# dohlee/rosettafold-pytorch

Measured on AMD Instinct MI355X. Metric: residues/sec forward (L=256, N=128), higher is better.
Workload: dtype bf16; 1 GPU; BASELINE.json configs[1]: bsz=4/GPU, n_seq=128, L=256, d_msa=384, d_pair=288, 8+5 blocks, 4 encoder layers, random-init weights; global_batch=4, parallelism=batch-sharded x1 (replicated weights), launch=one hipGraph replay per step (validation + input copy outside the graph)

## Files before the change

### rosettafold-pytorch_amd/csrc/favor.hip

```cpp
#include <type_traits>

#include "common.h"

#define FV_DH 64
#define FV_M 266
#define FV_MT 17
#define FV_MPAD 288
#define FV_CTX_LD 592
#define FV_DT 5
#define FV_DROWS 80

struct FavorAttnP {
  const h16_t* qkv;
  const h16_t* pc;
  h16_t* out;
  int64_t x_b, x_o, x_s;
  int64_t x_h;
  int64_t o_b, o_o, o_s;
  int q_off, k_off, v_off;
  int n_o, n_h, nitems;
  int nchunks;
  int dbg;
  float eps;
  float ctx_scale;
};

#ifdef RF_H16_IS_F16
#define FV_CS(x) ((x) * p.ctx_scale)
#else
#define FV_CS(x) (x)
#endif

typedef __attribute__((ext_vector_type(4))) short s16x4;

__device__ __forceinline__ int swz_off(int row, int chunk) { return row * 128 + ((chunk ^ (row & 7)) << 4); }

__device__ __forceinline__ void fv_load_tile(char* smem, int lds_off, const h16_t* g, int64_t stride, int nrows,
                                             int wave, int lane) {
  const int ninstr = nrows * 8 / 64;
  for (int it = wave; it < ninstr; it += 4) {
    const int slot = it * 64 + lane;
    const int row = slot >> 3;
    const int clog = (slot & 7) ^ (row & 7);
    rf_glds16(g + (int64_t)row * stride + clog * 8, smem + lds_off + it * 1024);
  }
}

__device__ __forceinline__ float rbf(float x) { return h2f(f2h(x)); }

__device__ __forceinline__ float fv_mfma_done(float acc_reg) {
  asm volatile("s_nop 7\n\ts_nop 3" : "+v"(acc_reg));
  return acc_reg;
}

union Frag {
  h16x8 v;
  unsigned u[4];
  uint2 h[2];
};

template <int LS, bool SOFTMAX>
__global__ __launch_bounds__(256, 1) void favor_attention_kernel(const FavorAttnP p) {
  constexpr int ST = LS / 64;
  constexpr int NSB = LS / 32;
  constexpr int PC_OFF = 0;
  constexpr int K_OFF = FV_MPAD * 128;
  constexpr int V_OFF = K_OFF + LS * 128;
  constexpr int CTX_OFF = V_OFF + LS * 128;
  constexpr int DIAG_OFF = CTX_OFF + FV_DROWS * FV_CTX_LD;
  constexpr int RED_OFF = DIAG_OFF + LS * 4;
  extern __shared__ __attribute__((aligned(16))) char smem[];
  const int tid = threadIdx.x, lane = tid & 63;
  const int wave = __builtin_amdgcn_readfirstlane(tid >> 6) & 3;
  const int fr = lane & 15, fq = lane >> 4;
  const int nm = wave == 0 ? 5 : 4;
  const int m0t = wave == 0 ? 0 : 5 + 4 * (wave - 1);
  const f32x4 epsv = {p.eps, p.eps, p.eps, p.eps};
  Frag ones;
#pragma unroll
  for (int k = 0; k < 4; ++k) ones.u[k] = fr == 0 ? RF_H16_ONE2 : 0u;

  fv_load_tile(smem, PC_OFF, p.pc, FV_DH, FV_MPAD, wave, lane);
  for (int i = tid; i < FV_DROWS * FV_CTX_LD / 4; i += 256) ((unsigned*)(smem + CTX_OFF))[i] = 0u;

  auto item_base = [&](int item, int64_t& xb, int64_t& ob) {
    const int h = item % p.n_h;
    const int t = item / p.n_h;
    const int o = t % p.n_o, b = t / p.n_o;
    xb = (int64_t)b * p.x_b + (int64_t)o * p.x_o + (int64_t)h * p.x_h;
    ob = (int64_t)b * p.o_b + (int64_t)o * p.o_o + h * FV_DH;
  };

  const int nch = p.nchunks;
  int item = blockIdx.x;
  if (item < p.nitems) {
    int64_t xb, ob;
    item_base(item, xb, ob);
    fv_load_tile(smem, K_OFF, p.qkv + xb + p.k_off, p.x_s, LS, wave, lane);
    fv_load_tile(smem, V_OFF, p.qkv + xb + p.v_off, p.x_s, LS, wave, lane);
  }
  bool first = true;
  for (; item < p.nitems; item += gridDim.x) {
    int64_t xb, ob;
    item_base(item, xb, ob);
    if (first)
      asm volatile("s_waitcnt vmcnt(0)" ::: "memory");
    else
      asm volatile("s_waitcnt vmcnt(%0)" ::"n"(ST * 4) : "memory");
    first = false;
    __syncthreads();
    h16x8 qf[ST][2];
    auto load_q = [&](int chunk) {
#pragma unroll
      for (int t = 0; t < ST; ++t) {
        const int s = chunk * LS + (wave * ST + t) * 16 + fr;
        const h16_t* qrow = p.qkv + xb + p.q_off + (int64_t)s * p.x_s;
#pragma unroll
        for (int kk = 0; kk < 2; ++kk) qf[t][kk] = *(const h16x8*)(qrow + (kk * 4 + fq) * 8);
      }
    };
    load_q(0);

    float gmax = 0.f;
    if constexpr (SOFTMAX) {
      for (int s = tid; s < LS; s += 256) {
        float a = 0.f;
#pragma unroll
        for (int c = 0; c < 8; ++c) {
          const h16x8 x = *(const h16x8*)(smem + K_OFF + s * 128 + c * 16);
#pragma unroll
          for (int e = 0; e < 8; ++e) {
            const float f = h2f((h16_t)x[e]);
            a = fmaf(f, f, a);
          }
        }
        ((float*)(smem + DIAG_OFF))[s] = a * (0.0625f * 1.4426950408889634f);
      }
    }

    h16x8 pf[5][2];
#pragma unroll
    for (int j = 0; j < 5; ++j)
#pragma unroll
      for (int kk = 0; kk < 2; ++kk)
        if (j < nm) pf[j][kk] = *(const h16x8*)(smem + PC_OFF + swz_off((m0t + j) * 16 + fr, kk * 4 + fq));

    if constexpr (SOFTMAX) {
      float mx = -INFINITY;
      for (int u = 0; u < NSB; ++u) {
        h16x8 kf[2][2];
#pragma unroll
        for (int t = 0; t < 2; ++t)
#pragma unroll
          for (int kk = 0; kk < 2; ++kk)
            kf[t][kk] = *(const h16x8*)(smem + K_OFF + swz_off((2 * u + t) * 16 + fr, kk * 4 + fq));
#pragma unroll
        for (int j = 0; j < 5; ++j) {
          if (j < nm) {
            const bool valid = (m0t + j) * 16 + fr < FV_M;
#pragma unroll
            for (int t = 0; t < 2; ++t) {
              f32x4 a = {0.f, 0.f, 0.f, 0.f};
              a = rf_mfma16(kf[t][0], pf[j][0], a, 0, 0, 0);
              a = rf_mfma16(kf[t][1], pf[j][1], a, 0, 0, 0);
              if (valid) mx = fmaxf(mx, fmaxf(fmaxf(a[0], a[1]), fmaxf(a[2], a[3])));
            }
          }
        }
      }
      mx = wave_max(mx);
      if (lane == 0) ((float*)(smem + RED_OFF))[wave] = mx;
      __syncthreads();
      const float* red = (const float*)(smem + RED_OFF);
      gmax = fmaxf(fmaxf(red[0], red[1]), fmaxf(red[2], red[3]));
    }

    f32x4 ctx[5][FV_DT];
#pragma unroll
    for (int j = 0; j < 5; ++j)
#pragma unroll
      for (int i = 0; i < FV_DT; ++i) ctx[j][i] = (f32x4){0.f, 0.f, 0.f, 0.f};
    for (int ck = 0; ck < nch; ++ck) {
    if (ck > 0) {
      __syncthreads();
      fv_load_tile(smem, K_OFF, p.qkv + xb + p.k_off + (int64_t)ck * LS * p.x_s, p.x_s, LS, wave, lane);
      fv_load_tile(smem, V_OFF, p.qkv + xb + p.v_off + (int64_t)ck * LS * p.x_s, p.x_s, LS, wave, lane);
      asm volatile("s_waitcnt vmcnt(0)" ::: "memory");
      __syncthreads();
    }
    for (int u = 0; u < NSB; ++u) {
      h16x8 kf[2][2];
#pragma unroll
      for (int t = 0; t < 2; ++t)
#pragma unroll
        for (int kk = 0; kk < 2; ++kk)
          kf[t][kk] = *(const h16x8*)(smem + K_OFF + swz_off((2 * u + t) * 16 + fr, kk * 4 + fq));
      Frag vf[4];
      {
        const int p4 = fr & 3;
#pragma unroll
        for (int i = 0; i < 4; ++i) {
#pragma unroll
          for (int half = 0; half < 2; ++half) {
            const int row = u * 32 + half * 16 + 4 * fq + (fr >> 2);
            const int off = V_OFF + swz_off(row, i * 2 + (p4 >> 1)) + (p4 & 1) * 8;
            const s16x4 r = __builtin_amdgcn_ds_read_tr16_b64_v4i16((__attribute__((address_space(3))) s16x4*)(smem + off));
            vf[i].h[half] = __builtin_bit_cast(uint2, r);
          }
        }
      }
      f32x4 init[2] = {epsv, epsv};
      if constexpr (SOFTMAX) {
#pragma unroll
        for (int t = 0; t < 2; ++t) {
          const float4 d4 = *(const float4*)(smem + DIAG_OFF + ((2 * u + t) * 16 + 4 * fq) * 4);
          init[t] = (f32x4){-(d4.x + gmax), -(d4.y + gmax), -(d4.z + gmax), -(d4.w + gmax)};
        }
      }
#pragma unroll
      for (int j = 0; j < 5; ++j) {
        if (j < nm) {
          f32x4 a[2];
#pragma unroll
          for (int t = 0; t < 2; ++t) {
            a[t] = rf_mfma16(kf[t][0], pf[j][0], init[t], 0, 0, 0);
            a[t] = rf_mfma16(kf[t][1], pf[j][1], a[t], 0, 0, 0);
          }
          float f[2][4];
#pragma unroll
          for (int t = 0; t < 2; ++t)
#pragma unroll
            for (int r = 0; r < 4; ++r) {
              if constexpr (SOFTMAX)
                f[t][r] = __builtin_amdgcn_exp2f(a[t][r]) + p.eps;
              else
                f[t][r] = fmaxf(a[t][r], p.eps);
            }
          if ((m0t + j) == FV_MT - 1 && fr >= FV_M - 16 * (FV_MT - 1)) {
#pragma unroll
            for (int t = 0; t < 2; ++t)
#pragma unroll
              for (int r = 0; r < 4; ++r) f[t][r] = 0.f;
          }
          Frag kfr;
          kfr.u[0] = rf_pack2_h16(f[0][0], f[0][1]);
          kfr.u[1] = rf_pack2_h16(f[0][2], f[0][3]);
          kfr.u[2] = rf_pack2_h16(f[1][0], f[1][1]);
          kfr.u[3] = rf_pack2_h16(f[1][2], f[1][3]);
#pragma unroll
          for (int i = 0; i < 4; ++i)
            ctx[j][i] = rf_mfma16(kfr.v, vf[i].v, ctx[j][i], 0, 0, 0);
          ctx[j][4] = rf_mfma16(kfr.v, ones.v, ctx[j][4], 0, 0, 0);
        }
      }
    }
    }
#pragma unroll
    for (int j = 0; j < 5; ++j) {
      if (j < nm) {
#pragma unroll
        for (int i = 0; i < FV_DT; ++i) {
          uint2 w;
          w.x = rf_pack2_h16(FV_CS(ctx[j][i][0]), FV_CS(ctx[j][i][1]));
          w.y = rf_pack2_h16(FV_CS(ctx[j][i][2]), FV_CS(ctx[j][i][3]));
          *(uint2*)(smem + CTX_OFF + (i * 16 + fr) * FV_CTX_LD + ((m0t + j) * 16 + 4 * fq) * 2) = w;
        }
      }
    }
    __syncthreads();

    asm volatile("s_waitcnt vmcnt(0)" ::: "memory");
    {
      const int nxt = item + gridDim.x;
      if (nxt < p.nitems) {
        int64_t xb2, ob2;
        item_base(nxt, xb2, ob2);
        fv_load_tile(smem, K_OFF, p.qkv + xb2 + p.k_off, p.x_s, LS, wave, lane);
        fv_load_tile(smem, V_OFF, p.qkv + xb2 + p.v_off, p.x_s, LS, wave, lane);
      }
    }

    f32x4 qinit[ST];
#pragma unroll
    for (int t = 0; t < ST; ++t) qinit[t] = epsv;
    if constexpr (SOFTMAX) {
      float dq[ST], rmax[ST];
#pragma unroll
      for (int t = 0; t < ST; ++t) {
        float a = 0.f;
#pragma unroll
        for (int kk = 0; kk < 2; ++kk)
#pragma unroll
          for (int e = 0; e < 8; ++e) {
            const float f = h2f((h16_t)qf[t][kk][e]);
            a = fmaf(f, f, a);
          }
        a += __shfl_xor(a, 16, 64);
        a += __shfl_xor(a, 32, 64);
        dq[t] = a * (0.0625f * 1.4426950408889634f);
        rmax[t] = -INFINITY;
      }
      for (int j = 0; j < FV_MT; ++j) {
        h16x8 pfr[2];
#pragma unroll
        for (int kk = 0; kk < 2; ++kk) pfr[kk] = *(const h16x8*)(smem + PC_OFF + swz_off(j * 16 + fr, kk * 4 + fq));
#pragma unroll
        for (int t = 0; t < ST; ++t) {
          f32x4 a = {0.f, 0.f, 0.f, 0.f};
          a = rf_mfma16(pfr[0], qf[t][0], a, 0, 0, 0);
          a = rf_mfma16(pfr[1], qf[t][1], a, 0, 0, 0);
#pragma unroll
          for (int r = 0; r < 4; ++r)
            if (j * 16 + 4 * fq + r < FV_M) rmax[t] = fmaxf(rmax[t], a[r]);
        }
      }
#pragma unroll
      for (int t = 0; t < ST; ++t) {
        rmax[t] = fmaxf(rmax[t], __shfl_xor(rmax[t], 16, 64));
        rmax[t] = fmaxf(rmax[t], __shfl_xor(rmax[t], 32, 64));
        const float off = -(dq[t] + rmax[t]);
        qinit[t] = (f32x4){off, off, off, off};
      }
    }
    for (int qc = 0; qc < nch; ++qc) {
    if (qc > 0) load_q(qc);
    f32x4 num[FV_DT][ST];
#pragma unroll
    for (int t = 0; t < ST; ++t)
#pragma unroll
      for (int i = 0; i < FV_DT; ++i) num[i][t] = (f32x4){0.f, 0.f, 0.f, 0.f};
    auto mblock = [&](int u, auto last_tag) {
      constexpr bool LAST = decltype(last_tag)::value;
      float f[2][ST][4];
#pragma unroll
      for (int jj = 0; jj < 2; ++jj) {
        if (LAST && jj == 1) {
#pragma unroll
          for (int t = 0; t < ST; ++t)
#pragma unroll
            for (int r = 0; r < 4; ++r) f[jj][t][r] = 0.f;
        } else {
          const int j = 2 * u + jj;
          h16x8 pfr[2];
#pragma unroll
          for (int kk = 0; kk < 2; ++kk) pfr[kk] = *(const h16x8*)(smem + PC_OFF + swz_off(j * 16 + fr, kk * 4 + fq));
#pragma unroll
          for (int t = 0; t < ST; ++t) {
            f32x4 a = rf_mfma16(pfr[0], qf[t][0], qinit[t], 0, 0, 0);
            a = rf_mfma16(pfr[1], qf[t][1], a, 0, 0, 0);
#pragma unroll
            for (int r = 0; r < 4; ++r) {
              float x;
              if constexpr (SOFTMAX)
                x = __builtin_amdgcn_exp2f(a[r]) + p.eps;
              else
                x = fmaxf(a[r], p.eps);
              if (LAST && 4 * fq + r >= FV_M - 16 * (FV_MT - 1)) x = 0.f;
              f[jj][t][r] = x;
            }
          }
        }
      }
      Frag cf[FV_DT];
#pragma unroll
      for (int i = 0; i < FV_DT; ++i) {
        const char* base = smem + CTX_OFF + (i * 16 + fr) * FV_CTX_LD + (32 * u + 4 * fq) * 2;
        cf[i].h[0] = *(const uint2*)base;
        cf[i].h[1] = *(const uint2*)(base + 32);
      }
#pragma unroll
      for (int t = 0; t < ST; ++t) {
        Frag qfr;
        qfr.u[0] = rf_pack2_h16(f[0][t][0], f[0][t][1]);
        qfr.u[1] = rf_pack2_h16(f[0][t][2], f[0][t][3]);
        qfr.u[2] = rf_pack2_h16(f[1][t][0], f[1][t][1]);
        qfr.u[3] = rf_pack2_h16(f[1][t][2], f[1][t][3]);
#pragma unroll
        for (int i = 0; i < FV_DT; ++i)
          num[i][t] = rf_mfma16(cf[i].v, qfr.v, num[i][t], 0, 0, 0);
      }
    };
    for (int u = 0; u < (FV_MT - 1) / 2; ++u) mblock(u, std::false_type{});
    mblock((FV_MT - 1) / 2, std::true_type{});
#pragma unroll
    for (int t = 0; t < ST; ++t) {
      const float dn = __shfl(fv_mfma_done(num[4][t][0]), fr, 64);
      const float inv = 1.f / dn;
      const int s = qc * LS + (wave * ST + t) * 16 + fr;
      h16_t* orow = p.out + ob + (int64_t)s * p.o_s;
#pragma unroll
      for (int i = 0; i < 4; ++i) {
        uint2 w;
        w.x = rf_pack2_h16(num[i][t][0] * inv, num[i][t][1] * inv);
        w.y = rf_pack2_h16(num[i][t][2] * inv, num[i][t][3] * inv);
        *(uint2*)(orow + i * 16 + 4 * fq) = w;
      }
    }
    }
  }
}

#pragma clang diagnostic ignored "-Winline-asm"
__device__ __forceinline__ void fv_glds_asm(const void* src, unsigned lds_addr) {
  asm volatile("s_mov_b32 m0, %0\n\ts_nop 0\n\tglobal_load_lds_dwordx4 %1, off" ::"s"(lds_addr), "v"(src) : "memory", "m0");
}

__device__ __forceinline__ void fv_lds_barrier() {
  asm volatile("s_waitcnt lgkmcnt(0)" ::: "memory");
  __builtin_amdgcn_s_barrier();
  asm volatile("" ::: "memory");
}

__device__ unsigned long long g_fv_cycles[8];
#define FV_STAMP(slot)                                                   \
  if (prof) {                                                            \
    const unsigned long long now = __builtin_readcyclecounter();         \
    acc_cyc[slot] += now - t_last;                                       \
    t_last = now;                                                        \
  }

template <int LS, bool SOFTMAX>
__global__ __launch_bounds__(512, 1) void favor_attention_kernel8(const FavorAttnP p) {
  constexpr int NSB = LS / 32;
  constexpr int NJ = 3;
  constexpr int STB = LS >= 128 ? LS / 128 : 1;
  constexpr int NWB = LS / (16 * STB);
  constexpr int PC_OFF = 0;
  constexpr int K_OFF = FV_MPAD * 128;
  constexpr int V_OFF = K_OFF + LS * 128;
  constexpr int CTX_OFF = V_OFF + LS * 128;
  constexpr int DIAG_OFF = CTX_OFF + FV_DROWS * FV_CTX_LD;
  constexpr int RED_OFF = DIAG_OFF + LS * 4;
  extern __shared__ __attribute__((aligned(16))) char smem[];
  const int tid = threadIdx.x, lane = tid & 63;
  const int wave = __builtin_amdgcn_readfirstlane(tid >> 6) & 7;
  const int fr = lane & 15, fq = lane >> 4;
  const int nm = wave == 0 ? 3 : 2;
  const int m0t = wave == 0 ? 0 : 1 + 2 * wave;
  const f32x4 epsv = {p.eps, p.eps, p.eps, p.eps};
  Frag ones;
#pragma unroll
  for (int k = 0; k < 4; ++k) ones.u[k] = fr == 0 ? RF_H16_ONE2 : 0u;

  const unsigned lds_base = (unsigned)(uintptr_t)(__attribute__((address_space(3))) char*)smem;
  auto load_tile8 = [&](int lds_off, const h16_t* gp, int64_t stride, auto nrows_tag) {
    constexpr int NI = decltype(nrows_tag)::value * 8 / 64;
    int ln = lane;
    asm volatile("" : "+v"(ln));
    const int dma_row = ln >> 3;
    const int dma_col = ((ln & 7) ^ dma_row) * 8;
    const h16_t* g0 = gp + (int64_t)dma_row * stride + dma_col;
#pragma unroll
    for (int k = 0; k < (NI + 7) / 8; ++k) {
      const int it = wave + 8 * k;
      if (NI % 8 == 0 || it < NI)
        fv_glds_asm(g0 + (int64_t)(8 * it) * stride, __builtin_amdgcn_readfirstlane(lds_base + lds_off + it * 1024));
    }
  };
  constexpr std::integral_constant<int, LS> LS_TAG{};
  load_tile8(PC_OFF, p.pc, FV_DH, std::integral_constant<int, FV_MPAD>{});
  for (int i = tid; i < FV_DROWS * FV_CTX_LD / 4; i += 512) ((unsigned*)(smem + CTX_OFF))[i] = 0u;

  auto item_base = [&](int item, int64_t& xb, int64_t& ob) {
    const int h = item % p.n_h;
    const int t = item / p.n_h;
    const int o = t % p.n_o, b = t / p.n_o;
    xb = (int64_t)b * p.x_b + (int64_t)o * p.x_o + (int64_t)h * p.x_h;
    ob = (int64_t)b * p.o_b + (int64_t)o * p.o_o + h * FV_DH;
  };
  auto ctx_col = [](int tile, int q4) { return ((tile >> 1) * 32 + 8 * q4 + 4 * (tile & 1)) * 2; };
  const int nch = SOFTMAX ? 1 : p.nchunks;
  int item = blockIdx.x;
  if (item < p.nitems) {
    int64_t xb, ob;
    item_base(item, xb, ob);
    load_tile8(K_OFF, p.qkv + xb + p.k_off, p.x_s, LS_TAG);
    load_tile8(V_OFF, p.qkv + xb + p.v_off, p.x_s, LS_TAG);
  }
  bool first = true;
  const bool prof = (RF_DBG(p.dbg) & 8) && wave == ((RF_DBG(p.dbg) >> 4) & 7);
  unsigned long long acc_cyc[7] = {0, 0, 0, 0, 0, 0, 0};
  unsigned long long t_last = prof ? __builtin_readcyclecounter() : 0;
  for (; item < p.nitems; item += gridDim.x) {
    int64_t xb, ob;
    item_base(item, xb, ob);
    asm volatile("" : "+v"(xb), "+v"(ob));
    if (prof) {
      t_last = __builtin_readcyclecounter();
      acc_cyc[6] += 1;
    }
    if (first || wave >= NWB)
      asm volatile("s_waitcnt vmcnt(0)" ::: "memory");
    else
      asm volatile("s_waitcnt vmcnt(%0)" ::"n"(STB * 4) : "memory");
    first = false;
    fv_lds_barrier();
    FV_STAMP(0)
    h16x8 pf[NJ][2];
    {
      int frP = fr, fqP = fq;
      asm volatile("" : "+v"(frP), "+v"(fqP));
#pragma unroll
      for (int j = 0; j < NJ; ++j)
#pragma unroll
        for (int kk = 0; kk < 2; ++kk)
          pf[j][kk] = *(const h16x8*)(smem + PC_OFF + m0t * 2048 + swz_off(frP, kk * 4 + fqP) + (j < nm ? j : 0) * 2048);
    }
    h16x8 qf[STB][2];
    auto load_q = [&](int chunk) {
      int frq = fr, fqq = fq;
      asm volatile("" : "+v"(frq), "+v"(fqq));
      if (wave < NWB) {
#pragma unroll
        for (int t = 0; t < STB; ++t) {
          const int s = chunk * LS + (wave * STB + t) * 16 + frq;
          const h16_t* qrow = p.qkv + xb + p.q_off + (int64_t)s * p.x_s;
#pragma unroll
          for (int kk = 0; kk < 2; ++kk) qf[t][kk] = *(const h16x8*)(qrow + (kk * 4 + fqq) * 8);
        }
      }
    };
    load_q(0);

    float gmax = 0.f;
    if constexpr (SOFTMAX) {
      int frS = fr, fqS = fq;
      asm volatile("" : "+v"(frS), "+v"(fqS));
      for (int s = tid; s < LS; s += 512) {
        float a = 0.f;
#pragma unroll
        for (int c = 0; c < 8; ++c) {
          const h16x8 x = *(const h16x8*)(smem + K_OFF + s * 128 + c * 16);
#pragma unroll
          for (int e = 0; e < 8; ++e) {
            const float f = h2f((h16_t)x[e]);
            a = fmaf(f, f, a);
          }
        }
        ((float*)(smem + DIAG_OFF))[s] = a * (0.0625f * 1.4426950408889634f);
      }
      float mx = -INFINITY;
      for (int u = 0; u < NSB; ++u) {
        h16x8 kf[2][2];
#pragma unroll
        for (int t = 0; t < 2; ++t)
#pragma unroll
          for (int kk = 0; kk < 2; ++kk)
            kf[t][kk] = *(const h16x8*)(smem + K_OFF + swz_off((2 * u + t) * 16 + frS, kk * 4 + fqS));
#pragma unroll
        for (int j = 0; j < NJ; ++j) {
          if (j < nm) {
            const h16x8* pfj = pf[j];
            const bool valid = (m0t + j) != FV_MT - 1 || frS < FV_M - 16 * (FV_MT - 1);
#pragma unroll
            for (int t = 0; t < 2; ++t) {
              f32x4 a = {0.f, 0.f, 0.f, 0.f};
              a = rf_mfma16(kf[t][0], pfj[0], a, 0, 0, 0);
              a = rf_mfma16(kf[t][1], pfj[1], a, 0, 0, 0);
              if (valid) mx = fmaxf(mx, fmaxf(fmaxf(a[0], a[1]), fmaxf(a[2], a[3])));
            }
          }
        }
      }
      mx = wave_max(mx);
      if (lane == 0) ((float*)(smem + RED_OFF))[wave] = mx;
      fv_lds_barrier();
      const float* red = (const float*)(smem + RED_OFF);
      gmax = fmaxf(fmaxf(fmaxf(red[0], red[1]), fmaxf(red[2], red[3])), fmaxf(fmaxf(red[4], red[5]), fmaxf(red[6], red[7])));
    }

    f32x4 ctx[NJ][FV_DT];
#pragma unroll
    for (int j = 0; j < NJ; ++j)
#pragma unroll
      for (int i = 0; i < FV_DT; ++i) ctx[j][i] = (f32x4){0.f, 0.f, 0.f, 0.f};
    for (int ck = 0; ck < nch; ++ck) {
      if (ck > 0) {
        __syncthreads();
        load_tile8(K_OFF, p.qkv + xb + p.k_off + (int64_t)ck * LS * p.x_s, p.x_s, LS_TAG);
        load_tile8(V_OFF, p.qkv + xb + p.v_off + (int64_t)ck * LS * p.x_s, p.x_s, LS_TAG);
        asm volatile("s_waitcnt vmcnt(0)" ::: "memory");
        __syncthreads();
      }
      h16x8 kf[2][2];
      Frag vf[4];
      auto load_sblock = [&](int u, h16x8 (&kfo)[2][2], Frag (&vfo)[4]) {
#pragma unroll
        for (int t = 0; t < 2; ++t)
#pragma unroll
          for (int kk = 0; kk < 2; ++kk)
            kfo[t][kk] = *(const h16x8*)(smem + K_OFF + swz_off((2 * u + t) * 16 + fr, kk * 4 + fq));
        const int p4 = fr & 3;
#pragma unroll
        for (int i = 0; i < 4; ++i) {
#pragma unroll
          for (int half = 0; half < 2; ++half) {
            const int row = u * 32 + half * 16 + 4 * fq + (fr >> 2);
            const int off = V_OFF + swz_off(row, i * 2 + (p4 >> 1)) + (p4 & 1) * 8;
            const s16x4 r = __builtin_amdgcn_ds_read_tr16_b64_v4i16((__attribute__((address_space(3))) s16x4*)(smem + off));
            vfo[i].h[half] = __builtin_bit_cast(uint2, r);
          }
        }
      };
      load_sblock(0, kf, vf);
      for (int u = 0; u < ((RF_DBG(p.dbg) & 1) ? 0 : NSB); ++u) {
        h16x8 kfn[2][2];
        Frag vfn[4];
        load_sblock(u + 1 < NSB ? u + 1 : u, kfn, vfn);
        f32x4 init[2] = {epsv, epsv};
        if constexpr (SOFTMAX) {
#pragma unroll
          for (int t = 0; t < 2; ++t) {
            const float4 d4 = *(const float4*)(smem + DIAG_OFF + ((2 * u + t) * 16 + 4 * fq) * 4);
            init[t] = (f32x4){-(d4.x + gmax), -(d4.y + gmax), -(d4.z + gmax), -(d4.w + gmax)};
          }
        }
#pragma unroll
        for (int j = 0; j < NJ; ++j) {
          if (j < nm) {
            const h16x8* pfj = pf[j];
            f32x4 a[2];
#pragma unroll
            for (int t = 0; t < 2; ++t) {
              a[t] = rf_mfma16(kf[t][0], pfj[0], init[t], 0, 0, 0);
              a[t] = rf_mfma16(kf[t][1], pfj[1], a[t], 0, 0, 0);
            }
            float f[2][4];
#pragma unroll
            for (int t = 0; t < 2; ++t)
#pragma unroll
              for (int r = 0; r < 4; ++r) {
                if constexpr (SOFTMAX)
                  f[t][r] = __builtin_amdgcn_exp2f(a[t][r]) + p.eps;
                else
                  f[t][r] = fmaxf(a[t][r], p.eps);
              }
            if ((m0t + j) == FV_MT - 1 && fr >= FV_M - 16 * (FV_MT - 1)) {
#pragma unroll
              for (int t = 0; t < 2; ++t)
#pragma unroll
                for (int r = 0; r < 4; ++r) f[t][r] = 0.f;
            }
            Frag kfr;
            kfr.u[0] = rf_pack2_h16(f[0][0], f[0][1]);
            kfr.u[1] = rf_pack2_h16(f[0][2], f[0][3]);
            kfr.u[2] = rf_pack2_h16(f[1][0], f[1][1]);
            kfr.u[3] = rf_pack2_h16(f[1][2], f[1][3]);
#pragma unroll
            for (int i = 0; i < 4; ++i)
              ctx[j][i] = rf_mfma16(kfr.v, vf[i].v, ctx[j][i], 0, 0, 0);
            ctx[j][4] = rf_mfma16(kfr.v, ones.v, ctx[j][4], 0, 0, 0);
          }
        }
#pragma unroll
        for (int t = 0; t < 2; ++t)
#pragma unroll
          for (int kk = 0; kk < 2; ++kk) kf[t][kk] = kfn[t][kk];
#pragma unroll
        for (int i = 0; i < 4; ++i) vf[i] = vfn[i];
      }
    }
    FV_STAMP(1)
#pragma unroll
    for (int j = 0; j < NJ; ++j)
      if (j < nm) {
#pragma unroll
        for (int i = 0; i < FV_DT; ++i) {
          uint2 w;
          w.x = rf_pack2_h16(FV_CS(ctx[j][i][0]), FV_CS(ctx[j][i][1]));
          w.y = rf_pack2_h16(FV_CS(ctx[j][i][2]), FV_CS(ctx[j][i][3]));
          *(uint2*)(smem + CTX_OFF + (i * 16 + fr) * FV_CTX_LD + ctx_col(m0t + j, fq)) = w;
        }
      }
    fv_lds_barrier();
    FV_STAMP(2)
    asm volatile("s_waitcnt vmcnt(0)" ::: "memory");
#pragma unroll
    for (int t = 0; t < STB; ++t) {
      asm volatile("" : "+v"(qf[t][0]), "+v"(qf[t][1]));
    }
    {
      const int nxt = item + gridDim.x;
      if (nxt < p.nitems) {
        int64_t xb2, ob2;
        item_base(nxt, xb2, ob2);
        load_tile8(K_OFF, p.qkv + xb2 + p.k_off, p.x_s, LS_TAG);
        load_tile8(V_OFF, p.qkv + xb2 + p.v_off, p.x_s, LS_TAG);
      }
    }
    FV_STAMP(3)
    for (int qc = 0; qc < nch; ++qc) {
      if (qc > 0) {
        load_q(qc);
        asm volatile("s_waitcnt vmcnt(0)" ::: "memory");
#pragma unroll
        for (int t = 0; t < STB; ++t) {
          asm volatile("" : "+v"(qf[t][0]), "+v"(qf[t][1]));
        }
      }
      if (wave < NWB) {
        f32x4 qinit[STB];
#pragma unroll
        for (int t = 0; t < STB; ++t) qinit[t] = epsv;
        if constexpr (SOFTMAX) {
          float dq[STB], rmax[STB];
#pragma unroll
          for (int t = 0; t < STB; ++t) {
            float a = 0.f;
#pragma unroll
            for (int kk = 0; kk < 2; ++kk)
#pragma unroll
              for (int e = 0; e < 8; ++e) {
                const float f = h2f((h16_t)qf[t][kk][e]);
                a = fmaf(f, f, a);
              }
            a += __shfl_xor(a, 16, 64);
            a += __shfl_xor(a, 32, 64);
            dq[t] = a * (0.0625f * 1.4426950408889634f);
            rmax[t] = -INFINITY;
          }
          for (int j = 0; j < FV_MT; ++j) {
            h16x8 pfr[2];
#pragma unroll
            for (int kk = 0; kk < 2; ++kk) pfr[kk] = *(const h16x8*)(smem + PC_OFF + swz_off(j * 16 + fr, kk * 4 + fq));
#pragma unroll
            for (int t = 0; t < STB; ++t) {
              f32x4 a = {0.f, 0.f, 0.f, 0.f};
              a = rf_mfma16(pfr[0], qf[t][0], a, 0, 0, 0);
              a = rf_mfma16(pfr[1], qf[t][1], a, 0, 0, 0);
#pragma unroll
              for (int r = 0; r < 4; ++r)
                if (j * 16 + 4 * fq + r < FV_M) rmax[t] = fmaxf(rmax[t], a[r]);
            }
          }
#pragma unroll
          for (int t = 0; t < STB; ++t) {
            rmax[t] = fmaxf(rmax[t], __shfl_xor(rmax[t], 16, 64));
            rmax[t] = fmaxf(rmax[t], __shfl_xor(rmax[t], 32, 64));
            const float off = -(dq[t] + rmax[t]);
            qinit[t] = (f32x4){off, off, off, off};
          }
        }
        f32x4 num[FV_DT][STB];
#pragma unroll
        for (int t = 0; t < STB; ++t)
#pragma unroll
          for (int i = 0; i < FV_DT; ++i) num[i][t] = (f32x4){0.f, 0.f, 0.f, 0.f};
        auto mblock = [&](int u, auto last_tag) {
          constexpr bool LAST = decltype(last_tag)::value;
          float f[2][STB][4];
#pragma unroll
          for (int jj = 0; jj < 2; ++jj) {
            if (LAST && jj == 1) {
#pragma unroll
              for (int t = 0; t < STB; ++t)
#pragma unroll
                for (int r = 0; r < 4; ++r) f[jj][t][r] = 0.f;
            } else {
              const int j = 2 * u + jj;
              h16x8 pfr[2];
#pragma unroll
              for (int kk = 0; kk < 2; ++kk) pfr[kk] = *(const h16x8*)(smem + PC_OFF + swz_off(j * 16 + fr, kk * 4 + fq));
#pragma unroll
              for (int t = 0; t < STB; ++t) {
                f32x4 a = rf_mfma16(pfr[0], qf[t][0], qinit[t], 0, 0, 0);
                a = rf_mfma16(pfr[1], qf[t][1], a, 0, 0, 0);
#pragma unroll
                for (int r = 0; r < 4; ++r) {
                  float x;
                  if constexpr (SOFTMAX)
                    x = __builtin_amdgcn_exp2f(a[r]) + p.eps;
                  else
                    x = fmaxf(a[r], p.eps);
                  if (LAST && 4 * fq + r >= FV_M - 16 * (FV_MT - 1)) x = 0.f;
                  f[jj][t][r] = x;
                }
              }
            }
          }
          Frag cf[FV_DT];
#pragma unroll
          for (int i = 0; i < FV_DT; ++i)
            cf[i].v = *(const h16x8*)(smem + CTX_OFF + (i * 16 + fr) * FV_CTX_LD + (32 * u + 8 * fq) * 2);
#pragma unroll
          for (int t = 0; t < STB; ++t) {
            Frag qfr;
            qfr.u[0] = rf_pack2_h16(f[0][t][0], f[0][t][1]);
            qfr.u[1] = rf_pack2_h16(f[0][t][2], f[0][t][3]);
            qfr.u[2] = rf_pack2_h16(f[1][t][0], f[1][t][1]);
            qfr.u[3] = rf_pack2_h16(f[1][t][2], f[1][t][3]);
#pragma unroll
            for (int i = 0; i < FV_DT; ++i)
              num[i][t] = rf_mfma16(cf[i].v, qfr.v, num[i][t], 0, 0, 0);
          }
        };
        for (int u = 0; u < ((RF_DBG(p.dbg) & 2) ? 0 : (FV_MT - 1) / 2); ++u) mblock(u, std::false_type{});
        mblock((FV_MT - 1) / 2, std::true_type{});
        FV_STAMP(4)
#pragma unroll
        for (int t = 0; t < STB; ++t) {
          const float dn = __shfl(fv_mfma_done(num[4][t][0]), fr, 64);
          const float inv = 1.f / dn;
          const int s = qc * LS + (wave * STB + t) * 16 + fr;
          h16_t* orow = p.out + ob + (int64_t)s * p.o_s;
#pragma unroll
          for (int i = 0; i < 4; ++i) {
            uint2 w;
            w.x = rf_pack2_h16(num[i][t][0] * inv, num[i][t][1] * inv);
            w.y = rf_pack2_h16(num[i][t][2] * inv, num[i][t][3] * inv);
            *(uint2*)(orow + i * 16 + 4 * fq) = w;
          }
        }
      }
    }
    FV_STAMP(5)
  }
  if (prof && lane == 0) {
#pragma unroll
    for (int i = 0; i < 7; ++i) atomicAdd(&g_fv_cycles[i], acc_cyc[i]);
  }
}

extern "C" int rf_favor_phase_cycles(unsigned long long* out7, int reset) {
  unsigned long long z[8] = {0, 0, 0, 0, 0, 0, 0, 0};
  if (out7 && hipMemcpyFromSymbol(out7, HIP_SYMBOL(g_fv_cycles), 7 * sizeof(unsigned long long)) != hipSuccess) return 1000 + (int)hipGetLastError();
  if (reset && hipMemcpyToSymbol(HIP_SYMBOL(g_fv_cycles), z, sizeof(z)) != hipSuccess) return 1000 + (int)hipGetLastError();
  return 0;
}

template <int LS, bool SM>
static int launch_favor(const FavorAttnP& p, hipStream_t s) {
  const size_t lds = (size_t)FV_MPAD * 128 + 2 * (size_t)LS * 128 + (size_t)FV_DROWS * FV_CTX_LD + LS * 4 + 64;
  const int ncu = rf_num_cus() > 0 ? rf_num_cus() : 256;
  const int grid = p.nitems < ncu ? p.nitems : ncu;
  static const bool force4 = getenv("RF_FAVOR4") != nullptr;
  constexpr bool only4 = SM && LS > 128;
  if (only4 || force4) {
    auto k = favor_attention_kernel<LS, SM>;
    if (const int e = rf_enable_big_lds<favor_attention_kernel<LS, SM>>()) return e;
    hipLaunchKernelGGL(k, dim3(grid), dim3(256), lds, s, p);
  } else if constexpr (!only4) {
    auto k = favor_attention_kernel8<LS, SM>;
    if (const int e = rf_enable_big_lds<favor_attention_kernel8<LS, SM>>()) return e;
    hipLaunchKernelGGL(k, dim3(grid), dim3(512), lds, s, p);
  }
  return rf_launch_status();
}

extern "C" int rf_favor_attention(const void* qkv, const void* pc, void* out, const int64_t x_strides[4],
                                  const int64_t o_strides[3], int q_off, int k_off, int v_off, int n_b, int n_o,
                                  int n_h, int seq_len, int dim_head, int n_features, int softmax_kernel, float eps,
                                  void* stream) {
  if (dim_head != FV_DH || n_features != FV_M) return RF_EINVAL;
  int nchunks = 1, ls = seq_len;
  if (seq_len > 256) {
    if (softmax_kernel || seq_len % 256) return RF_EINVAL;
    nchunks = seq_len / 256;
    ls = 256;
  }
  if (ls != 64 && ls != 128 && ls != 256) return RF_EINVAL;
  if (((uintptr_t)qkv % 16) || ((uintptr_t)pc % 16) || ((uintptr_t)out % 8)) return RF_EALIGN;
  for (int i = 0; i < 3; ++i)
    if (x_strides[i] % 8 || o_strides[i] % 4) return RF_EALIGN;
  if (x_strides[3] % 8) return RF_EALIGN;
  if (q_off % 8 || k_off % 8 || v_off % 8) return RF_EALIGN;
  FavorAttnP p;
  p.qkv = (const h16_t*)qkv;
  p.pc = (const h16_t*)pc;
  p.out = (h16_t*)out;
  p.x_b = x_strides[0]; p.x_o = x_strides[1]; p.x_s = x_strides[2]; p.x_h = x_strides[3];
  p.o_b = o_strides[0]; p.o_o = o_strides[1]; p.o_s = o_strides[2];
  p.q_off = q_off; p.k_off = k_off; p.v_off = v_off;
  p.n_o = n_o; p.n_h = n_h;
  p.nitems = n_b * n_o * n_h;
  p.eps = eps;
  p.nchunks = nchunks;
  p.ctx_scale = 1.0f;
#ifdef RF_H16_IS_F16
  for (int n = 1; n < seq_len; n <<= 1) p.ctx_scale *= 0.5f;
#endif
  static int dbg = 0;
  static const int dbg_rc = rf_dbg_env("RF_FAVOR_DBG", &dbg);
  if (dbg_rc) return dbg_rc;
  p.dbg = dbg;
  hipStream_t s = (hipStream_t)stream;
  if (ls == 256) return softmax_kernel ? launch_favor<256, true>(p, s) : launch_favor<256, false>(p, s);
  if (ls == 128) return softmax_kernel ? launch_favor<128, true>(p, s) : launch_favor<128, false>(p, s);
  return softmax_kernel ? launch_favor<64, true>(p, s) : launch_favor<64, false>(p, s);
}
```

Before: 3199 residues/s.

## Cache softmax-path random-feature logits in registers instead of recomputing MFMAs

In the softmax (FAVOR+ positive features) path, the key-side logits computed during the max-finding pass are now kept in registers (zk) and reused in the context accumulation, so the second set of key projection MFMAs is dropped. The query side likewise keeps its logits (zq) from the row-max pass and reuses them in the numerator loop, which is fully unrolled with compile-time indices. The key diagonal norm computation is also spread across 8 lanes per row with shuffle reductions. The softmax branch now handles only a single chunk and no longer contains the multi-chunk reload loop. The cost is much higher register pressure from the large cached accumulator arrays, which could cause spills or lower occupancy.

```diff
diff --git a/rosettafold-pytorch_amd/csrc/favor.hip b/rosettafold-pytorch_amd/csrc/favor.hip
--- a/rosettafold-pytorch_amd/csrc/favor.hip
+++ b/rosettafold-pytorch_amd/csrc/favor.hip
@@ -1,4 +1,5 @@
 #include <type_traits>
+#include <utility>
 
 #include "common.h"
 
@@ -51,6 +52,11 @@
 __device__ __forceinline__ float fv_mfma_done(float acc_reg) {
   asm volatile("s_nop 7\n\ts_nop 3" : "+v"(acc_reg));
   return acc_reg;
+}
+
+template <int... I, class F>
+__device__ __forceinline__ void fv_static_for(std::integer_sequence<int, I...>, F&& f) {
+  (f(std::integral_constant<int, I>{}), ...);
 }
 
 union Frag {
@@ -522,142 +528,205 @@
     };
     load_q(0);
 
-    float gmax = 0.f;
+    f32x4 ctx[NJ][FV_DT];
+#pragma unroll
+    for (int j = 0; j < NJ; ++j)
+#pragma unroll
+      for (int i = 0; i < FV_DT; ++i) ctx[j][i] = (f32x4){0.f, 0.f, 0.f, 0.f};
+    auto load_kblock = [&](int u, int frK, int fqK, h16x8 (&kfo)[2][2]) {
+#pragma unroll
+      for (int t = 0; t < 2; ++t)
+#pragma unroll
+        for (int kk = 0; kk < 2; ++kk)
+          kfo[t][kk] = *(const h16x8*)(smem + K_OFF + swz_off((2 * u + t) * 16 + frK, kk * 4 + fqK));
+    };
+    auto load_vblock = [&](int u, Frag (&vfo)[4]) {
+      const int p4 = fr & 3;
+#pragma unroll
+      for (int i = 0; i < 4; ++i) {
+#pragma unroll
+        for (int half = 0; half < 2; ++half) {
+          const int row = u * 32 + half * 16 + 4 * fq + (fr >> 2);
+          const int off = V_OFF + swz_off(row, i * 2 + (p4 >> 1)) + (p4 & 1) * 8;
+          const s16x4 r = __builtin_amdgcn_ds_read_tr16_b64_v4i16((__attribute__((address_space(3))) s16x4*)(smem + off));
+          vfo[i].h[half] = __builtin_bit_cast(uint2, r);
+        }
+      }
+    };
+    auto ctx_step = [&](int j, float (&f)[2][4], const Frag (&vfu)[4]) {
+      if ((m0t + j) == FV_MT - 1 && fr >= FV_M - 16 * (FV_MT - 1)) {
+#pragma unroll
+        for (int t = 0; t < 2; ++t)
+#pragma unroll
+          for (int r = 0; r < 4; ++r) f[t][r] = 0.f;
+      }
+      Frag kfr;
+      kfr.u[0] = rf_pack2_h16(f[0][0], f[0][1]);
+      kfr.u[1] = rf_pack2_h16(f[0][2], f[0][3]);
+      kfr.u[2] = rf_pack2_h16(f[1][0], f[1][1]);
+      kfr.u[3] = rf_pack2_h16(f[1][2], f[1][3]);
+#pragma unroll
+      for (int i = 0; i < 4; ++i)
+        ctx[j][i] = rf_mfma16(kfr.v, vfu[i].v, ctx[j][i], 0, 0, 0);
+      ctx[j][4] = rf_mfma16(kfr.v, ones.v, ctx[j][4], 0, 0, 0);
+    };
     if constexpr (SOFTMAX) {
-      int frS = fr, fqS = fq;
-      asm volatile("" : "+v"(frS), "+v"(fqS));
-      for (int s = tid; s < LS; s += 512) {
-        float a = 0.f;
-#pragma unroll
-        for (int c = 0; c < 8; ++c) {
-          const h16x8 x = *(const h16x8*)(smem + K_OFF + s * 128 + c * 16);
+      {
+        int tS = tid;
+        asm volatile("" : "+v"(tS));
+#pragma unroll
+        for (int r0 = 0; r0 < LS; r0 += 64) {
+          const int s = r0 + (tS >> 3);
+          const h16x8 x = *(const h16x8*)(smem + K_OFF + s * 128 + (tS & 7) * 16);
+          float a = 0.f;
 #pragma unroll
           for (int e = 0; e < 8; ++e) {
             const float f = h2f((h16_t)x[e]);
             a = fmaf(f, f, a);
           }
-        }
-        ((float*)(smem + DIAG_OFF))[s] = a * (0.0625f * 1.4426950408889634f);
-      }
+          a += __shfl_xor(a, 1, 64);
+          a += __shfl_xor(a, 2, 64);
+          a += __shfl_xor(a, 4, 64);
+          if ((tS & 7) == 0) ((float*)(smem + DIAG_OFF))[s] = a * (0.0625f * 1.4426950408889634f);
+        }
+      }
+      f32x4 zk[NJ][NSB][2];
+#pragma unroll
+      for (int j = 0; j < NJ; ++j)
+#pragma unroll
+        for (int u = 0; u < NSB; ++u)
+#pragma unroll
+          for (int t = 0; t < 2; ++t) zk[j][u][t] = (f32x4){0.f, 0.f, 0.f, 0.f};
       float mx = -INFINITY;
-      for (int u = 0; u < NSB; ++u) {
+      if (!(RF_DBG(p.dbg) & 1)) {
+        int frS = fr, fqS = fq;
+        asm volatile("" : "+v"(frS), "+v"(fqS));
+        auto logits = [&](int j, int u, const h16x8 (&kfu)[2][2]) {
+#pragma unroll
+          for (int t = 0; t < 2; ++t) {
+            zk[j][u][t] = rf_mfma16(kfu[t][0], pf[j][0], zk[j][u][t], 0, 0, 0);
+            zk[j][u][t] = rf_mfma16(kfu[t][1], pf[j][1], zk[j][u][t], 0, 0, 0);
+          }
+        };
+        auto track = [&](int j, int u) {
+          const bool valid = (m0t + j) != FV_MT - 1 || frS < FV_M - 16 * (FV_MT - 1);
+#pragma unroll
+          for (int t = 0; t < 2; ++t) {
+            const f32x4 a = zk[j][u][t];
+            const float m4 = fmaxf(fmaxf(a[0], a[1]), fmaxf(a[2], a[3]));
+            mx = valid ? fmaxf(mx, m4) : mx;
+          }
+        };
         h16x8 kf[2][2];
-#pragma unroll
-        for (int t = 0; t < 2; ++t)
-#pragma unroll
-          for (int kk = 0; kk < 2; ++kk)
-            kf[t][kk] = *(const h16x8*)(smem + K_OFF + swz_off((2 * u + t) * 16 + frS, kk * 4 + fqS));
-#pragma unroll
-        for (int j = 0; j < NJ; ++j) {
-          if (j < nm) {
-            const h16x8* pfj = pf[j];
-            const bool valid = (m0t + j) != FV_MT - 1 || frS < FV_M - 16 * (FV_MT - 1);
-#pragma unroll
-            for (int t = 0; t < 2; ++t) {
-              f32x4 a = {0.f, 0.f, 0.f, 0.f};
-              a = rf_mfma16(kf[t][0], pfj[0], a, 0, 0, 0);
-              a = rf_mfma16(kf[t][1], pfj[1], a, 0, 0, 0);
-              if (valid) mx = fmaxf(mx, fmaxf(fmaxf(a[0], a[1]), fmaxf(a[2], a[3])));
-            }
-          }
-        }
+        load_kblock(0, frS, fqS, kf);
+#pragma unroll
+        for (int u = 0; u < NSB; ++u) {
+          h16x8 kfn[2][2];
+          if (u + 1 < NSB) load_kblock(u + 1, frS, fqS, kfn);
+          logits(0, u, kf);
+          logits(1, u, kf);
+          if (u > 0) {
+            track(0, u - 1);
+            track(1, u - 1);
+          }
+          if (nm == 3) {
+            logits(2, u, kf);
+            if (u > 0) track(2, u - 1);
+            if (u == NSB - 1) track(2, u);
+          }
+          if (u + 1 < NSB) {
+#pragma unroll
+            for (int t = 0; t < 2; ++t)
+#pragma unroll
+              for (int kk = 0; kk < 2; ++kk) kf[t][kk] = kfn[t][kk];
+          }
+        }
+        asm volatile("s_nop 7\n\ts_nop 3"
+                     : "+v"(zk[0][NSB - 1][0]), "+v"(zk[0][NSB - 1][1]), "+v"(zk[1][NSB - 1][0]), "+v"(zk[1][NSB - 1][1]));
+        track(0, NSB - 1);
+        track(1, NSB - 1);
       }
       mx = wave_max(mx);
       if (lane == 0) ((float*)(smem + RED_OFF))[wave] = mx;
       fv_lds_barrier();
       const float* red = (const float*)(smem + RED_OFF);
-      gmax = fmaxf(fmaxf(fmaxf(red[0], red[1]), fmaxf(red[2], red[3])), fmaxf(fmaxf(red[4], red[5]), fmaxf(red[6], red[7])));
-    }
-
-    f32x4 ctx[NJ][FV_DT];
-#pragma unroll
-    for (int j = 0; j < NJ; ++j)
-#pragma unroll
-      for (int i = 0; i < FV_DT; ++i) ctx[j][i] = (f32x4){0.f, 0.f, 0.f, 0.f};
-    for (int ck = 0; ck < nch; ++ck) {
-      if (ck > 0) {
-        __syncthreads();
-        load_tile8(K_OFF, p.qkv + xb + p.k_off + (int64_t)ck * LS * p.x_s, p.x_s, LS_TAG);
-        load_tile8(V_OFF, p.qkv + xb + p.v_off + (int64_t)ck * LS * p.x_s, p.x_s, LS_TAG);
-        asm volatile("s_waitcnt vmcnt(0)" ::: "memory");
-        __syncthreads();
-      }
-      h16x8 kf[2][2];
-      Frag vf[4];
-      auto load_sblock = [&](int u, h16x8 (&kfo)[2][2], Frag (&vfo)[4]) {
-#pragma unroll
-        for (int t = 0; t < 2; ++t)
-#pragma unroll
-          for (int kk = 0; kk < 2; ++kk)
-            kfo[t][kk] = *(const h16x8*)(smem + K_OFF + swz_off((2 * u + t) * 16 + fr, kk * 4 + fq));
-        const int p4 = fr & 3;
-#pragma unroll
-        for (int i = 0; i < 4; ++i) {
-#pragma unroll
-          for (int half = 0; half < 2; ++half) {
-            const int row = u * 32 + half * 16 + 4 * fq + (fr >> 2);
-            const int off = V_OFF + swz_off(row, i * 2 + (p4 >> 1)) + (p4 & 1) * 8;
-            const s16x4 r = __builtin_amdgcn_ds_read_tr16_b64_v4i16((__attribute__((address_space(3))) s16x4*)(smem + off));
-            vfo[i].h[half] = __builtin_bit_cast(uint2, r);
-          }
-        }
-      };
-      load_sblock(0, kf, vf);
-      for (int u = 0; u < ((RF_DBG(p.dbg) & 1) ? 0 : NSB); ++u) {
-        h16x8 kfn[2][2];
-        Frag vfn[4];
-        load_sblock(u + 1 < NSB ? u + 1 : u, kfn, vfn);
-        f32x4 init[2] = {epsv, epsv};
-        if constexpr (SOFTMAX) {
+      const float gmax = fmaxf(fmaxf(fmaxf(red[0], red[1]), fmaxf(red[2], red[3])), fmaxf(fmaxf(red[4], red[5]), fmaxf(red[6], red[7])));
+      if (!(RF_DBG(p.dbg) & 1)) {
+        auto kmap = [&](int j, int u, const float (&off)[2][4], const Frag (&vfu)[4]) {
+          float f[2][4];
+#pragma unroll
+          for (int t = 0; t < 2; ++t)
+#pragma unroll
+            for (int r = 0; r < 4; ++r) f[t][r] = __builtin_amdgcn_exp2f(zk[j][u][t][r] + off[t][r]) + p.eps;
+          ctx_step(j, f, vfu);
+        };
+        Frag vf[4];
+        load_vblock(0, vf);
+#pragma unroll
+        for (int u = 0; u < NSB; ++u) {
+          Frag vfn[4];
+          if (u + 1 < NSB) load_vblock(u + 1, vfn);
+          float off[2][4];
 #pragma unroll
           for (int t = 0; t < 2; ++t) {
             const float4 d4 = *(const float4*)(smem + DIAG_OFF + ((2 * u + t) * 16 + 4 * fq) * 4);
-            init[t] = (f32x4){-(d4.x + gmax), -(d4.y + gmax), -(d4.z + gmax), -(d4.w + gmax)};
-          }
-        }
-#pragma unroll
-        for (int j = 0; j < NJ; ++j) {
-          if (j < nm) {
-            const h16x8* pfj = pf[j];
-            f32x4 a[2];
-#pragma unroll
-            for (int t = 0; t < 2; ++t) {
-              a[t] = rf_mfma16(kf[t][0], pfj[0], init[t], 0, 0, 0);
-              a[t] = rf_mfma16(kf[t][1], pfj[1], a[t], 0, 0, 0);
+            off[t][0] = -(d4.x + gmax);
+            off[t][1] = -(d4.y + gmax);
+            off[t][2] = -(d4.z + gmax);
+            off[t][3] = -(d4.w + gmax);
+          }
+          kmap(0, u, off, vf);
+          kmap(1, u, off, vf);
+          if (nm == 3) kmap(2, u, off, vf);
+          if (u + 1 < NSB) {
+#pragma unroll
+            for (int i = 0; i < 4; ++i) vf[i] = vfn[i];
+          }
+        }
+      }
+    } else {
+      for (int ck = 0; ck < nch; ++ck) {
+        if (ck > 0) {
+          __syncthreads();
+          load_tile8(K_OFF, p.qkv + xb + p.k_off + (int64_t)ck * LS * p.x_s, p.x_s, LS_TAG);
+          load_tile8(V_OFF, p.qkv + xb + p.v_off + (int64_t)ck * LS * p.x_s, p.x_s, LS_TAG);
+          asm volatile("s_waitcnt vmcnt(0)" ::: "memory");
+          __syncthreads();
+        }
+        h16x8 kf[2][2];
+        Frag vf[4];
+        load_kblock(0, fr, fq, kf);
+        load_vblock(0, vf);
+        for (int u = 0; u < ((RF_DBG(p.dbg) & 1) ? 0 : NSB); ++u) {
+          h16x8 kfn[2][2];
+          Frag vfn[4];
+          load_kblock(u + 1 < NSB ? u + 1 : u, fr, fq, kfn);
+          load_vblock(u + 1 < NSB ? u + 1 : u, vfn);
+#pragma unroll
+          for (int j = 0; j < NJ; ++j) {
+            if (j < nm) {
+              const h16x8* pfj = pf[j];
+              f32x4 a[2];
+#pragma unroll
+              for (int t = 0; t < 2; ++t) {
+                a[t] = rf_mfma16(kf[t][0], pfj[0], epsv, 0, 0, 0);
+                a[t] = rf_mfma16(kf[t][1], pfj[1], a[t], 0, 0, 0);
+              }
+              float f[2][4];
+#pragma unroll
+              for (int t = 0; t < 2; ++t)
+#pragma unroll
+                for (int r = 0; r < 4; ++r) f[t][r] = fmaxf(a[t][r], p.eps);
+              ctx_step(j, f, vf);
             }
-            float f[2][4];
-#pragma unroll
-            for (int t = 0; t < 2; ++t)
-#pragma unroll
-              for (int r = 0; r < 4; ++r) {
-                if constexpr (SOFTMAX)
-                  f[t][r] = __builtin_amdgcn_exp2f(a[t][r]) + p.eps;
-                else
-                  f[t][r] = fmaxf(a[t][r], p.eps);
-              }
-            if ((m0t + j) == FV_MT - 1 && fr >= FV_M - 16 * (FV_MT - 1)) {
-#pragma unroll
-              for (int t = 0; t < 2; ++t)
-#pragma unroll
-                for (int r = 0; r < 4; ++r) f[t][r] = 0.f;
-            }
-            Frag kfr;
-            kfr.u[0] = rf_pack2_h16(f[0][0], f[0][1]);
-            kfr.u[1] = rf_pack2_h16(f[0][2], f[0][3]);
-            kfr.u[2] = rf_pack2_h16(f[1][0], f[1][1]);
-            kfr.u[3] = rf_pack2_h16(f[1][2], f[1][3]);
-#pragma unroll
-            for (int i = 0; i < 4; ++i)
-              ctx[j][i] = rf_mfma16(kfr.v, vf[i].v, ctx[j][i], 0, 0, 0);
-            ctx[j][4] = rf_mfma16(kfr.v, ones.v, ctx[j][4], 0, 0, 0);
-          }
-        }
-#pragma unroll
-        for (int t = 0; t < 2; ++t)
-#pragma unroll
-          for (int kk = 0; kk < 2; ++kk) kf[t][kk] = kfn[t][kk];
-#pragma unroll
-        for (int i = 0; i < 4; ++i) vf[i] = vfn[i];
+          }
+#pragma unroll
+          for (int t = 0; t < 2; ++t)
+#pragma unroll
+            for (int kk = 0; kk < 2; ++kk) kf[t][kk] = kfn[t][kk];
+#pragma unroll
+          for (int i = 0; i < 4; ++i) vf[i] = vfn[i];
+        }
       }
     }
     FV_STAMP(1)
@@ -702,6 +771,7 @@
         f32x4 qinit[STB];
 #pragma unroll
         for (int t = 0; t < STB; ++t) qinit[t] = epsv;
+        f32x4 zq[SOFTMAX ? FV_MT : 1][STB];
         if constexpr (SOFTMAX) {
           float dq[STB], rmax[STB];
 #pragma unroll
@@ -719,20 +789,24 @@
             dq[t] = a * (0.0625f * 1.4426950408889634f);
             rmax[t] = -INFINITY;
           }
+#pragma unroll
           for (int j = 0; j < FV_MT; ++j) {
             h16x8 pfr[2];
 #pragma unroll
             for (int kk = 0; kk < 2; ++kk) pfr[kk] = *(const h16x8*)(smem + PC_OFF + swz_off(j * 16 + fr, kk * 4 + fq));
 #pragma unroll
             for (int t = 0; t < STB; ++t) {
-              f32x4 a = {0.f, 0.f, 0.f, 0.f};
-              a = rf_mfma16(pfr[0], qf[t][0], a, 0, 0, 0);
-              a = rf_mfma16(pfr[1], qf[t][1], a, 0, 0, 0);
+              zq[j][t] = rf_mfma16(pfr[0], qf[t][0], (f32x4){0.f, 0.f, 0.f, 0.f}, 0, 0, 0);
+              zq[j][t] = rf_mfma16(pfr[1], qf[t][1], zq[j][t], 0, 0, 0);
+            }
+          }
+#pragma unroll
+          for (int j = 0; j < FV_MT; ++j)
+#pragma unroll
+            for (int t = 0; t < STB; ++t)
 #pragma unroll
               for (int r = 0; r < 4; ++r)
-                if (j * 16 + 4 * fq + r < FV_M) rmax[t] = fmaxf(rmax[t], a[r]);
-            }
-          }
+                if (j * 16 + 4 * fq + r < FV_M) rmax[t] = fmaxf(rmax[t], zq[j][t][r]);
 #pragma unroll
           for (int t = 0; t < STB; ++t) {
             rmax[t] = fmaxf(rmax[t], __shfl_xor(rmax[t], 16, 64));
@@ -746,7 +820,7 @@
         for (int t = 0; t < STB; ++t)
 #pragma unroll
           for (int i = 0; i < FV_DT; ++i) num[i][t] = (f32x4){0.f, 0.f, 0.f, 0.f};
-        auto mblock = [&](int u, auto last_tag) {
+        auto mblock = [&](auto u, auto last_tag) {
           constexpr bool LAST = decltype(last_tag)::value;
           float f[2][STB][4];
 #pragma unroll
@@ -759,12 +833,19 @@
             } else {
               const int j = 2 * u + jj;
               h16x8 pfr[2];
-#pragma unroll
-              for (int kk = 0; kk < 2; ++kk) pfr[kk] = *(const h16x8*)(smem + PC_OFF + swz_off(j * 16 + fr, kk * 4 + fq));
+              if constexpr (!SOFTMAX) {
+#pragma unroll
+                for (int kk = 0; kk < 2; ++kk) pfr[kk] = *(const h16x8*)(smem + PC_OFF + swz_off(j * 16 + fr, kk * 4 + fq));
+              }
 #pragma unroll
               for (int t = 0; t < STB; ++t) {
-                f32x4 a = rf_mfma16(pfr[0], qf[t][0], qinit[t], 0, 0, 0);
-                a = rf_mfma16(pfr[1], qf[t][1], a, 0, 0, 0);
+                f32x4 a;
+                if constexpr (SOFTMAX) {
+                  a = zq[j][t] + qinit[t];
+                } else {
+                  a = rf_mfma16(pfr[0], qf[t][0], qinit[t], 0, 0, 0);
+                  a = rf_mfma16(pfr[1], qf[t][1], a, 0, 0, 0);
+                }
 #pragma unroll
                 for (int r = 0; r < 4; ++r) {
                   float x;
@@ -794,8 +875,13 @@
               num[i][t] = rf_mfma16(cf[i].v, qfr.v, num[i][t], 0, 0, 0);
           }
         };
-        for (int u = 0; u < ((RF_DBG(p.dbg) & 2) ? 0 : (FV_MT - 1) / 2); ++u) mblock(u, std::false_type{});
-        mblock((FV_MT - 1) / 2, std::true_type{});
+        if constexpr (SOFTMAX) {
+          if (!(RF_DBG(p.dbg) & 2))
+            fv_static_for(std::make_integer_sequence<int, (FV_MT - 1) / 2>{}, [&](auto u) { mblock(u, std::false_type{}); });
+        } else {
+          for (int u = 0; u < ((RF_DBG(p.dbg) & 2) ? 0 : (FV_MT - 1) / 2); ++u) mblock(u, std::false_type{});
+        }
+        mblock(std::integral_constant<int, (FV_MT - 1) / 2>{}, std::true_type{});
         FV_STAMP(4)
 #pragma unroll
         for (int t = 0; t < STB; ++t) {
```

Result: no change. 3219 residues/s (median of 2 runs) (+0.6%).
